# MAC-VO/MAC-VO

Measured on NVIDIA H100. Metric: stereo frames/sec @640x480, higher is better.
Workload: dtype f32

## Files before the change

include/macvo_b200.h:

```cpp
#ifndef MACVO_B200_H
#define MACVO_B200_H

#include <stddef.h>
#include <stdint.h>

#ifdef __cplusplus
extern "C" {
#endif

#define MACVO_OK 0
#define MACVO_E_ARG (-1)
#define MACVO_E_WORKSPACE (-2)
#define MACVO_E_UNSUPPORTED (-3)
#define MACVO_E_DRIVER (-4)

const char* macvo_b200_version(void);

#define MACVO_CORR_SIMT 0
#define MACVO_CORR_TC_3XF16 1
#define MACVO_CORR_TC_1XF16 2
#define MACVO_CORR_TC_TF32 3
#define MACVO_CORR_KMAJOR_INPUT 16
size_t macvo_corr_workspace_bytes(int batch, int dim, int n, int mode);
int macvo_corr_build(const float* fmap1, const float* fmap2, float* corr, int batch, int dim, int n, int mode,
// ... 50 lines not shown
                           float min_depth_cov, float match_cov_default, double* out_cov, float* out_point,
                           int* status, void* stream);

typedef struct {
    int max_steps;
    int patience;
    int max_reject;
    int cluster;
    double decreasing;
    double huber_delta;
    double radius;
    double diag_min;
    double diag_max;
} macvo_pgo_params_t;
int macvo_pgo_solve(const double* pos_Tw, const double* kp2_uv, const double* kp2_disp, const double* uv_cov,
                    const double* disp_cov, int k, const double* intr, double* pose_io,
                    const macvo_pgo_params_t* params, double* stats, void* stream);

#define MACVO_PGO_DISP 0
#define MACVO_PGO_REPROJ 1
#define MACVO_PGO_ICP 2
int macvo_pgo_solve_graph(int graph_type, const double* pos_Tw, const double* kp2_uv, const double* kp2_disp,
                          const double* uv_cov, const double* disp_cov, const double* pc_obs, const double* obs_cov,
                          const double* pts_cov, int k, const double* intr, double* pose_io,
                          const macvo_pgo_params_t* params, double* stats, void* stream);

int macvo_pgo_solve_counted(const double* pos_Tw, const double* kp2_uv, const double* kp2_disp, const double* uv_cov,
                            const double* disp_cov, int k_capacity, const int* k_dev, int min_k, const double* intr,
                            double* pose_io, const macvo_pgo_params_t* params, double* stats, void* stream,
                            int graph_type, const double* pc_obs, const double* obs_cov, const double* pts_cov);

size_t macvo_pgo_exchange_bytes(int world);
int macvo_p2p_alloc(size_t bytes, void** dev_ptr, unsigned char* ipc_handle64);
int macvo_p2p_open(const unsigned char* ipc_handle64, void** peer_ptr);
int macvo_p2p_close(void* peer_ptr);
int macvo_p2p_free(void* dev_ptr);
int macvo_pgo_solve_sharded(const double* pos_Tw, const double* kp2_uv, const double* kp2_disp, const double* uv_cov,
                            const double* disp_cov, int k_shard, const int* k_total_dev, int k_offset, int min_k,
                            const double* intr, double* pose_io, const macvo_pgo_params_t* params, double* stats,
                            void* const* exchange_bufs, int world, int rank, void* stream);

#define MACVO_PGO_ACC 55
#define MACVO_PGO_MAX_RANKS 8
int macvo_pgo_accumulate(const double* pos_Tw, const double* kp2_uv, const double* kp2_disp, const double* uv_cov,
                         const double* disp_cov, int k, const double* intr, const double* pose, double huber_delta,
                         double* acc, void* stream);

int macvo_layer_norm(const float* x, const float* weight, const float* bias, float* y, long long rows,
                     int channels, float eps, void* stream);
int macvo_add_layer_norm(const float* x, const float* resid, const float* weight, const float* bias, float* sum_out,
                         float* y, long long rows, int channels, float eps, void* stream);
int macvo_mlp_tc(const float* xn, const float* resid, const float* w1, const float* b1, const float* w2, const float* b2,
                 float* out, int rows, int channels, int hidden, void* stream);
int macvo_patch_embed_conv1(const float* maps, const float* weight, const float* bias, float* out,
                            long long n_maps, int h, int w, int allow_tf32, void* stream);
int macvo_add_rows_relu(float* x, const float* term, long long rows, int period, int channels, void* stream);
int macvo_small_attention(const float* q, const float* k, const float* v, float* out, int batch, int nq, int nk,
                          int heads, int head_dim, int q_broadcast, int allow_tf32, void* stream);

int macvo_small_attention_ex(const float* q, const float* k, const float* v, float* out, int batch, int nq, int nk,
                             int heads, int head_dim, int q_broadcast, int allow_tf32, int ldq, int ldk, int ldv,
                             const float* q_add, const float* k_add, int add_period, void* stream);

int macvo_latent_pool(const float* tokens, const float* ut, const float* wv, const float* bv, float* out,
                      long long n_maps, int nk, void* stream);

int macvo_gru_input(const float* mf, const float* agg, const float* gamma, float* buf0, float* buf1, float* buf2,
                    float* buf3, long long pixels, void* stream);
int macvo_gru_gates(const float* zr, const float* bias, const float* hx, float* z_out, float* rhx, long long pixels,
                    void* stream);
int macvo_gru_blend(const float* q, const float* bias, const float* z, float* hx, float* h_dense, long long pixels,
                    void* stream);
size_t macvo_rows_count(int batch, int height, int width, int vertical);
int macvo_conv_tc(const void* in_rows, int in_channels, int in_dense, const void* weights, const float* bias, int n_pad,
                  int n_valid, int ksize, int relu, int batch, int height, int width, void* out16, int out16_pitch,
                  int out16_offset, int out16_dense, float* out32, int out32_pitch, int out32_offset, int out32_planes,
                  void* stream);
int macvo_flow_im2col(const float* coords1, const float* coords0, void* rows, float* mf32, void* mf16_rows, int batch,
                      int height, int width, void* stream);

size_t macvo_gru_tc_operand_rows(int batch, int height, int width, int vertical);
int macvo_gru_tc_stage(int stage, int vertical, int batch, int height, int width, const void* h_rows, const void* x_rows,
                       const void* weights, const float* bias, float* h_master, float* z, void* out_rows, void* stream);
int macvo_gru_tc_pack(const float* src, int src_pitch, int channels, void* dst, int dst_channels, int dst_offset, int batch,
                      int height, int width, int vertical, void* stream);
int macvo_gru_tc_pack_motion(const float* mf, const float* agg, const float* gamma, void* x_rows_h, void* x_rows_v, int batch,
                             int height, int width, void* stream);
int macvo_softmax_rows_f16(const float* scores, void* out, long long rows, int cols, void* stream);
int macvo_convex_upsample(const float* flow, const float* mask_nhwc, float* out, float scale, int batch, int height, int width,
                          void* stream);

int macvo_cov_sanity_filter(const double* obs1_cov, const double* obs2_cov, int k, uint8_t* good, void* stream);
#define MACVO_COV_MATCH 0
#define MACVO_COV_IDENTITY 1
#define MACVO_COV_DIAGONALIZE 1
#define MACVO_COV_NORMALIZE 2
#define MACVO_COV_MAX_OPS 2
typedef struct {
    const float* depth_cov0;
    const float* depth_cov1;
    int simple_depth;
    float min_depth, max_depth;
    int front_of_cam;
    int icp;
    int cov_model;
    int cov_ops[MACVO_COV_MAX_OPS];
// ... 35 lines not shown
```

mac-vo_b200/build.py:

```python
from __future__ import annotations

import hashlib
import os
import shutil
import subprocess
import sys

PKG_DIR = os.path.dirname(os.path.abspath(__file__))
CSRC = os.path.join(PKG_DIR, "csrc")
LIB_DIR = os.path.join(PKG_DIR, "lib")
LIB_PATH = os.path.join(LIB_DIR, "libmacvo_b200.so")
SOURCES = ["corr_build.cu", "corr_build_simt.cu", "corr_build_tc.cu", "corr_lookup.cu", "dense_select.cu",
           "cov2to3.cu", "pgo.cu", "nn_kernels.cu", "decoder_fused.cu", "observe.cu", "decoder_token.cu", "motion_interp.cu",
           "gru_conv_tc.cu", "conv_tc.cu", "posenet.cu", "mlp_tc.cu"]
NVCC_FLAGS = ["-gencode", "arch=compute_90a,code=sm_90a", "-O3", "-lineinfo", "-std=c++17",
              "-Xcompiler", "-fPIC", "--use_fast_math=false"]


def _nvcc() -> str:
    for cand in (os.environ.get("NVCC"), shutil.which("nvcc"), "/usr/local/cuda/bin/nvcc"):
        if cand and os.path.exists(cand):
            return cand
    raise RuntimeError("nvcc not found (CUDA 12.9 toolkit expected at /usr/local/cuda)")


def _fingerprint() -> str:
    h = hashlib.sha256()
    for name in sorted(os.listdir(CSRC)) + ["../../include/macvo_b200.h"]:
        with open(os.path.join(CSRC, name), "rb") as f:
            h.update(name.encode())
            h.update(f.read())
    h.update(" ".join(NVCC_FLAGS).encode())
    return h.hexdigest()


def build(force: bool = False, verbose: bool = True) -> str:
    os.makedirs(LIB_DIR, exist_ok=True)
    stamp = os.path.join(LIB_DIR, "libmacvo_b200.stamp")
    fp = _fingerprint()
    if not force and os.path.exists(LIB_PATH) and os.path.exists(stamp) and open(stamp).read() == fp:
        return LIB_PATH
    nvcc = _nvcc()
    flags = [f for f in NVCC_FLAGS if f != "--use_fast_math=false"]
    objs = []
    procs = []
    for src in SOURCES:
        obj = os.path.join(LIB_DIR, src.replace(".cu", ".o"))
        objs.append(obj)
        cmd = [nvcc, *flags, "-c", os.path.join(CSRC, src), "-o", obj]
        procs.append((src, subprocess.Popen(cmd, stdout=subprocess.PIPE, stderr=subprocess.STDOUT, text=True)))
    for src, p in procs:
        out, _ = p.communicate()
        if p.returncode != 0:
            raise RuntimeError(f"nvcc failed on {src}:\n{out}")
        if verbose and out.strip():
            print(out, file=sys.stderr)
    link = [nvcc, "-shared", "-gencode", "arch=compute_90a,code=sm_90a", "-o", LIB_PATH, *objs, "-lcuda" if False else "-lcudart_static",
            "-Xlinker", "--no-undefined", "-lpthread", "-ldl", "-lrt"]
    r = subprocess.run(link, stdout=subprocess.PIPE, stderr=subprocess.STDOUT, text=True)
    if r.returncode != 0:
        raise RuntimeError(f"link failed:\n{r.stdout}")
    with open(stamp, "w") as f:
        f.write(fp)
    if verbose:
        print(f"built {LIB_PATH}", file=sys.stderr)
    return LIB_PATH

# ... 4 lines not shown
```

mac-vo_b200/csrc/nn_kernels.cu:

```cuda
#include "common.cuh"
#include <math_constants.h>

namespace {

__device__ __forceinline__ float2 ffma2_rn(float2 a, float2 b, float2 c) { return make_float2(fmaf(a.x, b.x, c.x), fmaf(a.y, b.y, c.y)); }
__device__ __forceinline__ float2 fmul2_rn(float2 a, float2 b) { return make_float2(__fmul_rn(a.x, b.x), __fmul_rn(a.y, b.y)); }

template <int VPL>
__global__ void __launch_bounds__(256)
layer_norm_kernel(const float* __restrict__ x, const float* __restrict__ w, const float* __restrict__ b,
                  float* __restrict__ y, long long rows, float eps, const float* __restrict__ resid = nullptr,
                  float* __restrict__ sum_out = nullptr) {
    constexpr int C = 32 * VPL;
    const long long row = (long long)blockIdx.x * 8 + (threadIdx.x >> 5);
    const int lane = threadIdx.x & 31;
    if (row >= rows) return;
    const float* xr = x + row * C;
    float v[VPL];
    float s = 0.f;
#pragma unroll
    for (int i = 0; i < VPL / 4; ++i) {
        float4 t = *reinterpret_cast<const float4*>(xr + (lane + 32 * i) * 4);
        if (resid) {
            const float4 r = *reinterpret_cast<const float4*>(resid + row * C + (lane + 32 * i) * 4);
            t = make_float4(t.x + r.x, t.y + r.y, t.z + r.z, t.w + r.w);
            *reinterpret_cast<float4*>(sum_out + row * C + (lane + 32 * i) * 4) = t;
        }
        v[4 * i] = t.x; v[4 * i + 1] = t.y; v[4 * i + 2] = t.z; v[4 * i + 3] = t.w;
        s += (t.x + t.y) + (t.z + t.w);
    }
    const float mean = warp_sum(s) * (1.f / C);
    float q = 0.f;
#pragma unroll
    for (int i = 0; i < VPL; ++i) { const float d = v[i] - mean; q = fmaf(d, d, q); }
    const float rstd = rsqrtf(warp_sum(q) * (1.f / C) + eps);
    float* yr = y + row * C;
#pragma unroll
    for (int i = 0; i < VPL / 4; ++i) {
        const int c = (lane + 32 * i) * 4;
        const float4 ww = *reinterpret_cast<const float4*>(w + c), bb = *reinterpret_cast<const float4*>(b + c);
        float4 o;
        o.x = (v[4 * i] - mean) * rstd * ww.x + bb.x;
        o.y = (v[4 * i + 1] - mean) * rstd * ww.y + bb.y;
        o.z = (v[4 * i + 2] - mean) * rstd * ww.z + bb.z;
        o.w = (v[4 * i + 3] - mean) * rstd * ww.w + bb.w;
        *reinterpret_cast<float4*>(yr + c) = o;
    }
}

__global__ void __launch_bounds__(256)
layer_norm64_kernel(const float* __restrict__ x, const float* __restrict__ w, const float* __restrict__ b,
                    float* __restrict__ y, long long rows, float eps) {
    const long long row = (long long)blockIdx.x * 8 + (threadIdx.x >> 5);
    const int lane = threadIdx.x & 31;
    if (row >= rows) return;
    const float2 t = *reinterpret_cast<const float2*>(x + row * 64 + lane * 2);
    const float mean = warp_sum(t.x + t.y) * (1.f / 64);
    const float d0 = t.x - mean, d1 = t.y - mean;
    const float rstd = rsqrtf(warp_sum(fmaf(d0, d0, d1 * d1)) * (1.f / 64) + eps);
    const float2 ww = *reinterpret_cast<const float2*>(w + lane * 2), bb = *reinterpret_cast<const float2*>(b + lane * 2);
    *reinterpret_cast<float2*>(y + row * 64 + lane * 2) = make_float2(d0 * rstd * ww.x + bb.x, d1 * rstd * ww.y + bb.y);
}

__global__ void __launch_bounds__(256)
add_rows_relu_kernel(float* __restrict__ x, const float* __restrict__ term, long long rows, int period, int c4) {
    const long long e = (long long)blockIdx.x * blockDim.x + threadIdx.x;
    if (e >= rows * c4) return;
    const long long r = e / c4;
    const int c = (int)(e % c4);
    float4 v = reinterpret_cast<float4*>(x)[e];
    const float4 t = __ldg(reinterpret_cast<const float4*>(term) + (r % period) * c4 + c);
    v.x = fmaxf(v.x + t.x, 0.f); v.y = fmaxf(v.y + t.y, 0.f); v.z = fmaxf(v.z + t.z, 0.f); v.w = fmaxf(v.w + t.w, 0.f);
    reinterpret_cast<float4*>(x)[e] = v;
}

constexpr int PE_C = 16, PE_K = 6;
__constant__ float c_pe_w[PE_K * PE_K * PE_C + PE_C];
__device__ float g_pe_pack[PE_K * PE_K * PE_C + PE_C];

__global__ void pe_pack_weights_kernel(const float* __restrict__ wgt, const float* __restrict__ bias, float* __restrict__ packed) {
    const int e = threadIdx.x + blockIdx.x * blockDim.x;
    if (e < PE_C * 36) { const int c = e / 36, t = e % 36; packed[t * PE_C + c] = wgt[e]; }
    else if (e < PE_C * 36 + PE_C) packed[e] = bias[e - PE_C * 36];
}

__global__ void __launch_bounds__(320)
patch_conv1_kernel(const float* __restrict__ maps, float* __restrict__ out, int h, int w, int ho, int wo) {
    extern __shared__ float sm[];
    float* s_map = sm;
    const int hp = 2 * ho + 4, wp = 2 * wo + 4;
    const float* src = maps + (long long)blockIdx.x * h * w;
    for (int e = threadIdx.x; e < hp * wp; e += blockDim.x) {
        const int y = e / wp - 2, x = e % wp - 2;
        s_map[e] = (y >= 0 && y < h && x >= 0 && x < w) ? __ldg(src + y * w + x) : 0.f;
    }
    __syncthreads();
    float* dst = out + (long long)blockIdx.x * ho * wo * PE_C;
    const int wo2 = wo >> 1;
    for (int p = threadIdx.x; p < ho * wo2; p += blockDim.x) {
        const int oy = p / wo2, ox = (p % wo2) * 2;
// ... 689 lines not shown
```

mac-vo_b200/flowformer_cov.py:

```python
from __future__ import annotations

import math
import os
import zlib
from typing import Callable

import torch
import torch.nn.functional as F

Tensor = torch.Tensor

LATENT_TOKENS = 8
LATENT_DIM = 128
QUERY_DIM = 64
COST_INPUT_DIM = 64
VERT_C_DIM = 64
ENCODER_DEPTH = 3


def _svt_spec(prefix: str) -> list[tuple[str, tuple[int, ...], str]]:
    out: list[tuple[str, tuple[int, ...], str]] = []
    dims, heads, srs, patch, cin = (128, 256), (4, 8), (8, 4), (4, 2), (3, 128)
    for s, (C, sr, ps, ci) in enumerate(zip(dims, srs, patch, cin)):
        p = f"{prefix}.svt."
# ... 312 lines not shown
        x = x.reshape(B, nh, nw, ws, ws, C).transpose(2, 3).reshape(B, nh * ws, nw * ws, C)
        return x[:, :H, :W, :].reshape(B, H * W, C)

    def _svt_local_attn(self, x: Tensor, size, p: str, heads: int, ws: int = 7) -> Tensor:
        B, N, C = x.shape
        H, W = size
        xw, meta = self._to_windows(x.view(B, H, W, C), ws)
        wq, bq = self.W[p + "qkv.weight"], self.W[p + "qkv.bias"]
        q, k, v = (F.linear(xw, wq[i * C:(i + 1) * C], bq[i * C:(i + 1) * C]) for i in range(3))
        o = self._attn(q, k, v, heads)
        return self._lin(self._from_windows(o, meta, ws, H, W), p + "proj")

    def _svt_global_attn(self, x: Tensor, size, p: str, heads: int, sr: int) -> Tensor:
        B, N, C = x.shape
        q = self._lin(x, p + "q")
        t = self._conv(x.permute(0, 2, 1).reshape(B, C, *size), p + "sr", stride=sr)
        t = self._ln(t.reshape(B, C, -1).permute(0, 2, 1), p + "norm")
        wkv, bkv = self.W[p + "kv.weight"], self.W[p + "kv.bias"]
        o = self._attn(q, F.linear(t, wkv[:C], bkv[:C]), F.linear(t, wkv[C:], bkv[C:]), heads)
        return self._lin(o, p + "proj")

    def patch_embed(self, cost_maps: Tensor) -> Tensor:
        p = "memory_encoder.cost_perceiver_encoder.patch_embed."
        M, _, H2, W2 = cost_maps.shape
        if self._native(cost_maps) and (H2 + 7) // 8 * 8 * ((W2 + 7) // 8 * 8) <= 96 * 160:
            if torch.backends.cudnn.allow_tf32:
                x = self._ops.patch_embed_conv1(cost_maps, self.W[p + "proj.0.weight"], self.W[p + "proj.0.bias"], s2d=True)
                w2 = self._memo(("pe_w2_s2d", x.device), lambda: self._ops.space_to_depth_filter(self.W[p + "proj.2.weight"])
                                .contiguous(memory_format=torch.channels_last))
                x = torch.cudnn_convolution_relu(x, w2, self.W[p + "proj.2.bias"], (1, 1), (1, 1), (1, 1), 1)
            else:
                x = self._ops.patch_embed_conv1(cost_maps, self.W[p + "proj.0.weight"], self.W[p + "proj.0.bias"])
                x = self._conv_relu(x, p + "proj.2", stride=2, padding=2)
        else:
            x = F.pad(cost_maps, (0, (8 - W2 % 8) % 8, 0, (8 - H2 % 8) % 8))
            x = self._conv_relu(x, p + "proj.0", stride=2, padding=2)
            x = self._conv_relu(x, p + "proj.2", stride=2, padding=2)
        native = self._native(x)
        x = F.conv2d(x if x.is_contiguous(memory_format=torch.channels_last) else x.contiguous(memory_format=torch.channels_last),
                     self.W[p + "proj.4.weight"], None if native else self.W[p + "proj.4.bias"], stride=2, padding=2)
        h, w = x.shape[2:]

        w0, b0 = self.W[p + "ffn_with_coord.0.weight"], self.W[p + "ffn_with_coord.0.bias"]

        def coord_term():
            xy = coords_grid(1, h, w, x.device, x.dtype) * 8 + 4
            enc = sine_embed(xy.view(1, 2, -1).permute(0, 2, 1), COST_INPUT_DIM)
            term = F.linear(enc, w0[:, COST_INPUT_DIM:, 0, 0], b0)
            if native:
                term = term + F.linear(self.W[p + "proj.4.bias"], w0[:, :COST_INPUT_DIM, 0, 0])
            return term.contiguous()
        term = self._memo(("pe", h, w, x.dtype, x.device, native), coord_term)
        t = x.permute(0, 2, 3, 1).reshape(M, h * w, COST_INPUT_DIM)
        t = F.linear(t, w0[:, :COST_INPUT_DIM, 0, 0])
        t = self._ops.add_rows_relu_(t, term[0]) if native else F.relu(t + term)
        t = F.linear(t, self.W[p + "ffn_with_coord.2.weight"][:, :, 0, 0], self.W[p + "ffn_with_coord.2.bias"])
        return self._ln(t, p + "norm")

    def _latent_layer(self, x: Tensor, p: str) -> Tensor:
        y = self._ln(x, p + "norm1")
        a = self._attn(self._lin(y, p + "q"), self._lin(y, p + "k"), self._lin(y, p + "v"), 8)
        x, xn = self._add_ln(x, self._lin(a, p + "proj"), p + "norm2")
        return self._mlp_residual(x, xn, p, "ffn.0", "ffn.3")

    def _context_tokens(self, context: Tensor, p: str, reps: int) -> Tensor:
        b, _, H, W = context.shape
        c = self._lin(context.flatten(2).permute(0, 2, 1), p + "context_proj").view(b, H, W, -1)
        return c.repeat(reps, 1, 1, 1)

    def _vert_local_attn_native(self, x: Tensor, size, context: Tensor, p: str, ws: int, heads: int) -> Tensor:
        Bt, N, C = x.shape
        H, W = size
        b = context.shape[0]
        wq, wk = self.W[p + "q.weight"], self.W[p + "k.weight"]
        enc = self._memo(("win", ws, C + VERT_C_DIM, x.dtype, x.device), lambda: sine_embed(
            coords_grid(1, ws, ws, x.device, x.dtype).view(1, 2, -1).permute(0, 2, 1), C + VERT_C_DIM))
        cproj = self._lin(context.flatten(2).permute(0, 2, 1), p + "context_proj").view(b, H, W, -1)
        cw, meta = self._to_windows(cproj, ws)
        w_qk_c = torch.cat([wq[:, C:], wk[:, C:]], 0)
        w_qk = torch.cat([wq, wk], 0)
        b_qk = torch.cat([self.W[p + "q.bias"], self.W[p + "k.bias"]], 0)
        terms = F.linear(cw, w_qk_c) + F.linear(enc, w_qk, b_qk)
        q_add, k_add = terms[..., :C].contiguous(), terms[..., C:].contiguous()
        w_x = self._memo(("vloc_w", p), lambda: torch.cat([wq[:, :C], wk[:, :C], self.W[p + "v.weight"]], 0).contiguous())
        b_x = self._memo(("vloc_b", p), lambda: torch.cat([torch.zeros(2 * C, device=x.device, dtype=x.dtype), self.W[p + "v.bias"]], 0))
        xw, meta = self._to_windows(x.view(Bt, H, W, C), ws)
        qkv = F.linear(xw, w_x, b_x)
        o = self._ops.fused_qkv_attention(qkv, heads, q_add, k_add)
        return self._lin(self._from_windows(o, meta, ws, H, W), p + "proj")

    def _vert_local_attn(self, x: Tensor, size, context: Tensor, p: str, ws: int = 7, heads: int = 8) -> Tensor:
        if self._native(x) and (x.shape[-1] // heads) in (16, 32):
            return self._vert_local_attn_native(x, size, context, p, ws, heads)
        Bt, N, C = x.shape
        H, W = size
        ctx = self._context_tokens(context, p, Bt // context.shape[0])
        xg = x.view(Bt, H, W, C)
        xw, meta = self._to_windows(xg, ws)
        qkw, _ = self._to_windows(torch.cat([xg, ctx], dim=-1), ws)
        enc = self._memo(("win", ws, C + VERT_C_DIM, x.dtype, x.device), lambda: sine_embed(
            coords_grid(1, ws, ws, x.device, x.dtype).view(1, 2, -1).permute(0, 2, 1), C + VERT_C_DIM))
        qkw = qkw + enc
        o = self._attn(self._lin(qkw, p + "q"), self._lin(qkw, p + "k"), self._lin(xw, p + "v"), heads)
        return self._lin(self._from_windows(o, meta, ws, H, W), p + "proj")

    def _vert_global_attn_native(self, x: Tensor, size, context: Tensor, p: str, sr: int, heads: int) -> Tensor:
        Bt, N, C = x.shape
        H, W = size
        b = context.shape[0]
# ... 414 lines not shown
```

mac-vo_b200/ops.py:

```python
from __future__ import annotations

import ctypes as C
import os
import threading

import torch

from .build import LIB_PATH

Tensor = torch.Tensor

CORR_SIMT, CORR_TC_3XF16, CORR_TC_1XF16, CORR_TC_TF32 = 0, 1, 2, 3
CORR_MODE_NAMES = {0: "simt", 1: "tc3", 2: "tc1", 3: "tf32"}
CORR_KMAJOR_INPUT = 16
PGO_ACC = 55

_lib = None
_lock = threading.Lock()
LAUNCHES = [0]


class MacvoB200Error(RuntimeError):
    pass

# ... 14 lines not shown
class _PgoParams(C.Structure):
    _fields_ = [("max_steps", C.c_int), ("patience", C.c_int), ("max_reject", C.c_int), ("cluster", C.c_int),
                ("decreasing", C.c_double), ("huber_delta", C.c_double), ("radius", C.c_double),
                ("diag_min", C.c_double), ("diag_max", C.c_double)]


EXPORTS = {
    "macvo_b200_version": (C.c_char_p, []),
    "macvo_corr_workspace_bytes": (C.c_size_t, [C.c_int] * 4),
    "macvo_corr_build": (C.c_int, [C.c_void_p] * 3 + [C.c_int] * 4 + [C.c_void_p, C.c_size_t, C.c_void_p]),
    "macvo_corr_lookup": (C.c_int, [C.c_void_p] * 3 + [C.c_int] * 5 + [C.c_void_p]),
    "macvo_corr_lookup_rows": (C.c_int, [C.c_void_p] * 3 + [C.c_int] * 5 + [C.c_void_p]),
    "macvo_dense_postproc": (C.c_int, [C.c_void_p] * 2 + [C.c_int] * 2 + [C.c_double] * 2 + [C.c_void_p] * 5
                             + [C.POINTER(_ScoreT), C.c_void_p]),
    "macvo_select_workspace_bytes": (C.c_size_t, [C.c_int] * 2),
    "macvo_select_candidates": (C.c_int, [C.c_void_p] * 5 + [C.c_int] * 3 + [C.c_double] + [C.c_void_p] * 5
                                + [C.c_size_t, C.c_void_p]),
    "macvo_select_candidates_depth": (C.c_int, [C.c_void_p] * 10 + [C.c_int] * 3 + [C.c_double] * 3 + [C.c_void_p] * 5
                                      + [C.c_size_t, C.c_void_p]),
    "macvo_select_mapping_candidates": (C.c_int, [C.c_void_p] * 2 + [C.c_int] * 3 + [C.c_float] * 2
                                        + [C.c_void_p] * 3 + [C.c_size_t, C.c_void_p]),
    "macvo_gather_pixels": (C.c_int, [C.c_void_p] * 2 + [C.c_int] * 2 + [C.c_void_p] * 2),
    "macvo_retrieve_pixels": (C.c_int, [C.c_void_p, C.c_int, C.c_int, C.c_void_p] + [C.c_int] * 3 + [C.c_void_p] * 2),
    "macvo_match_covariance": (C.c_int, [C.c_void_p, C.c_int, C.c_int, C.c_void_p, C.c_int, C.c_int, C.c_void_p,
                                         C.c_longlong, C.c_longlong, C.c_void_p]
                               + [C.c_float] * 4 + [C.c_int] + [C.c_float] * 3 + [C.c_void_p] * 4),
    "macvo_pgo_solve": (C.c_int, [C.c_void_p] * 5 + [C.c_int] + [C.c_void_p] * 2 + [C.POINTER(_PgoParams)]
                        + [C.c_void_p] * 2),
    "macvo_pgo_solve_graph": (C.c_int, [C.c_int] + [C.c_void_p] * 8 + [C.c_int] + [C.c_void_p] * 2 + [C.POINTER(_PgoParams)]
                              + [C.c_void_p] * 2),
    "macvo_pgo_solve_counted": (C.c_int, [C.c_void_p] * 5 + [C.c_int, C.c_void_p, C.c_int] + [C.c_void_p] * 2
                                + [C.POINTER(_PgoParams)] + [C.c_void_p] * 2 + [C.c_int] + [C.c_void_p] * 3),
    "macvo_motion_interpolate_workspace_bytes": (C.c_size_t, [C.c_int]),
    "macvo_motion_interpolate": (C.c_int, [C.c_void_p, C.c_void_p, C.c_int, C.c_void_p, C.c_void_p, C.c_size_t, C.c_void_p]),
    "macvo_cov_sanity_filter": (C.c_int, [C.c_void_p] * 2 + [C.c_int] + [C.c_void_p] * 2),
    "macvo_cov_modify": (C.c_int, [C.c_void_p, C.c_int, C.c_void_p, C.c_int, C.c_void_p]),
    "macvo_observe_workspace_bytes": (C.c_size_t, [C.c_int]),
    "macvo_observe_packed_doubles": (C.c_size_t, [C.c_int, C.c_int]),
    "macvo_observe_pack": (C.c_int, [C.c_void_p, C.c_int, C.c_int] + [C.c_void_p] * 6 + [C.c_int] * 3 + [C.c_void_p] * 2
                           + [C.c_int] + [C.c_float] * 3 + [C.c_void_p] * 6 + [C.c_size_t, C.c_void_p]
                           + [C.POINTER(_ObserveExt)]),
    "macvo_pgo_exchange_bytes": (C.c_size_t, [C.c_int]),
    "macvo_p2p_alloc": (C.c_int, [C.c_size_t, C.POINTER(C.c_void_p), C.c_char_p]),
    "macvo_p2p_open": (C.c_int, [C.c_char_p, C.POINTER(C.c_void_p)]),
    "macvo_p2p_close": (C.c_int, [C.c_void_p]),
    "macvo_p2p_free": (C.c_int, [C.c_void_p]),
    "macvo_pgo_solve_sharded": (C.c_int, [C.c_void_p] * 5 + [C.c_int, C.c_void_p, C.c_int, C.c_int] + [C.c_void_p] * 2
                                + [C.POINTER(_PgoParams)] + [C.c_void_p] * 2 + [C.c_int, C.c_int, C.c_void_p]),
    "macvo_pgo_accumulate": (C.c_int, [C.c_void_p] * 5 + [C.c_int] + [C.c_void_p] * 2 + [C.c_double]
                             + [C.c_void_p] * 2),
    "macvo_layer_norm": (C.c_int, [C.c_void_p] * 4 + [C.c_longlong, C.c_int, C.c_float, C.c_void_p]),
    "macvo_add_layer_norm": (C.c_int, [C.c_void_p] * 6 + [C.c_longlong, C.c_int, C.c_float, C.c_void_p]),
    "macvo_mlp_tc": (C.c_int, [C.c_void_p] * 7 + [C.c_int] * 3 + [C.c_void_p]),
    "macvo_patch_embed_conv1": (C.c_int, [C.c_void_p] * 4 + [C.c_longlong, C.c_int, C.c_int, C.c_int, C.c_void_p]),
    "macvo_add_rows_relu": (C.c_int, [C.c_void_p] * 2 + [C.c_longlong, C.c_int, C.c_int, C.c_void_p]),
    "macvo_small_attention": (C.c_int, [C.c_void_p] * 4 + [C.c_int] * 7 + [C.c_void_p]),
    "macvo_small_attention_ex": (C.c_int, [C.c_void_p] * 4 + [C.c_int] * 10 + [C.c_void_p] * 2 + [C.c_int, C.c_void_p]),
    "macvo_latent_pool": (C.c_int, [C.c_void_p] * 5 + [C.c_longlong, C.c_int, C.c_void_p]),
    "macvo_decoder_token_blob_floats": (C.c_size_t, []),
    "macvo_decoder_token": (C.c_int, [C.c_void_p] * 6 + [C.c_int, C.c_int, C.c_float, C.c_void_p]),
    "macvo_decoder_token_rows": (C.c_int, [C.c_void_p] * 6 + [C.c_int] * 3 + [C.c_float, C.c_void_p]),
    "macvo_gru_input": (C.c_int, [C.c_void_p] * 7 + [C.c_longlong, C.c_void_p]),
    "macvo_gru_gates": (C.c_int, [C.c_void_p] * 5 + [C.c_longlong, C.c_void_p]),
    "macvo_gru_blend": (C.c_int, [C.c_void_p] * 5 + [C.c_longlong, C.c_void_p]),
    "macvo_softmax_rows_f16": (C.c_int, [C.c_void_p] * 2 + [C.c_longlong, C.c_int, C.c_void_p]),
    "macvo_convex_upsample": (C.c_int, [C.c_void_p] * 3 + [C.c_float] + [C.c_int] * 3 + [C.c_void_p]),
    "macvo_rows_count": (C.c_size_t, [C.c_int] * 4),
    "macvo_conv_tc": (C.c_int, [C.c_void_p, C.c_int, C.c_int, C.c_void_p, C.c_void_p] + [C.c_int] * 7
                      + [C.c_void_p] + [C.c_int] * 3 + [C.c_void_p] + [C.c_int] * 3 + [C.c_void_p]),
    "macvo_flow_im2col": (C.c_int, [C.c_void_p] * 5 + [C.c_int] * 3 + [C.c_void_p]),
    "macvo_gru_tc_operand_rows": (C.c_size_t, [C.c_int] * 4),
    "macvo_gru_tc_stage": (C.c_int, [C.c_int] * 5 + [C.c_void_p] * 8),
    "macvo_gru_tc_pack": (C.c_int, [C.c_void_p, C.c_int, C.c_int, C.c_void_p] + [C.c_int] * 6 + [C.c_void_p]),
    "macvo_gru_tc_pack_motion": (C.c_int, [C.c_void_p] * 5 + [C.c_int] * 3 + [C.c_void_p]),
    "macvo_posenet_input": (C.c_int, [C.c_void_p] * 2 + [C.c_int] * 2 + [C.c_double, C.c_void_p, C.c_void_p]),
    "macvo_posenet_conv": (C.c_int, [C.c_void_p, C.c_int, C.c_int, C.c_int] + [C.c_void_p] * 2 + [C.c_int] * 5
                           + [C.c_void_p, C.c_int, C.c_void_p, C.c_void_p]),
    "macvo_posenet_head_floats": (C.c_size_t, []),
    "macvo_posenet_head": (C.c_int, [C.c_void_p] * 6),
}


def load_library(path: str | None = None):
    global _lib
    with _lock:
        if _lib is not None:
            return _lib
        path = path or os.environ.get("MACVO_B200_LIB", LIB_PATH)
        if not os.path.exists(path):
            raise MacvoB200Error(f"{path} not found: build it first with `python -m macvo_b200.build` "
                                 "(or __graft_entry__.build()); there is no CPU fallback")
        lib = C.CDLL(path)
        for name, (res, args) in EXPORTS.items():
            fn = getattr(lib, name)
            fn.restype, fn.argtypes = res, args
        _lib = lib
        return lib


def version() -> str:
    return load_library().macvo_b200_version().decode()


def _check(rc: int, what: str) -> None:
    if rc == 0:
        return
# ... 600 lines not shown
def layer_norm(x: Tensor, weight: Tensor, bias: Tensor, eps: float = 1e-5) -> Tensor:
    x = _dev(x, torch.float32, "layer_norm x")
    c = x.shape[-1]
    if c not in LAYER_NORM_CHANNELS:
        raise MacvoB200Error(f"layer_norm: channels {c} not in {LAYER_NORM_CHANNELS}")
    y = torch.empty_like(x)
    rc = load_library().macvo_layer_norm(x.data_ptr(), _dev(weight, torch.float32, "ln weight").data_ptr(),
                                         _dev(bias, torch.float32, "ln bias").data_ptr(), y.data_ptr(),
                                         x.numel() // c, c, float(eps), _stream())
    _check(rc, "macvo_layer_norm")
    LAUNCHES[0] += 1
    return y


def add_layer_norm(x: Tensor, resid: Tensor, weight: Tensor, bias: Tensor, eps: float = 1e-5) -> tuple[Tensor, Tensor]:
    x, resid = _dev(x, torch.float32, "add_layer_norm x"), _dev(resid, torch.float32, "add_layer_norm resid")
    c = x.shape[-1]
    if c not in (128, 256, 512) or x.shape != resid.shape:
        raise MacvoB200Error(f"add_layer_norm: channels {c} / shapes {tuple(x.shape)} vs {tuple(resid.shape)} unsupported")
    s, y = torch.empty_like(x), torch.empty_like(x)
    rc = load_library().macvo_add_layer_norm(x.data_ptr(), resid.data_ptr(), _dev(weight, torch.float32, "ln weight").data_ptr(),
                                             _dev(bias, torch.float32, "ln bias").data_ptr(), s.data_ptr(), y.data_ptr(),
                                             x.numel() // c, c, float(eps), _stream())
    _check(rc, "macvo_add_layer_norm")
    LAUNCHES[0] += 1
    return s, y


MLP_TC_HIDDEN = (128, 512)


def round_tf32(w: Tensor) -> Tensor:
    i = w.detach().to(torch.float32).contiguous().view(torch.int32)
    return ((i + 0xFFF + ((i >> 13) & 1)) & -0x2000).view(torch.float32)


def mlp_tc(xn: Tensor, resid: Tensor, w1: Tensor, b1: Tensor, w2: Tensor, b2: Tensor) -> Tensor:
    xn, resid = _dev(xn, torch.float32, "mlp_tc xn"), _dev(resid, torch.float32, "mlp_tc resid")
    w1, w2 = _dev(w1, torch.float32, "mlp_tc w1"), _dev(w2, torch.float32, "mlp_tc w2")
    b1, b2 = _dev(b1, torch.float32, "mlp_tc b1"), _dev(b2, torch.float32, "mlp_tc b2")
    c, hd = xn.shape[-1], w1.shape[0]
    if (c != 128 or hd not in MLP_TC_HIDDEN or xn.shape != resid.shape or tuple(w1.shape) != (hd, c)
            or tuple(w2.shape) != (c, hd) or b1.numel() != hd or b2.numel() != c):
        raise MacvoB200Error(f"mlp_tc: unsupported shapes xn {tuple(xn.shape)}, resid {tuple(resid.shape)}, "
                             f"w1 {tuple(w1.shape)}, w2 {tuple(w2.shape)}")
    out = torch.empty_like(resid)
    rc = load_library().macvo_mlp_tc(xn.data_ptr(), resid.data_ptr(), w1.data_ptr(), b1.data_ptr(), w2.data_ptr(),
                                      b2.data_ptr(), out.data_ptr(), xn.numel() // c, c, hd, _stream())
    _check(rc, "macvo_mlp_tc")
    LAUNCHES[0] += 1
    return out


def patch_embed_conv1(maps: Tensor, weight: Tensor, bias: Tensor, allow_tf32: bool | None = None, s2d: bool = False) -> Tensor:
    maps = _dev(maps, torch.float32, "patch_embed maps")
    m, one, h, w = maps.shape
    if one != 1 or tuple(weight.shape) != (16, 1, 6, 6):
        raise MacvoB200Error("patch_embed_conv1: expects (M,1,H,W) maps and a (16,1,6,6) weight")
    ho, wo = (h + 7) // 8 * 4, (w + 7) // 8 * 4
    tf32 = bool(torch.backends.cudnn.allow_tf32 if allow_tf32 is None else allow_tf32)
    if s2d and not tf32:
        raise MacvoB200Error("patch_embed_conv1: the space-to-depth output exists for the TF32 tensor-core variant only")
    out = torch.empty((m, ho // 2, wo // 2, 64) if s2d else (m, ho, wo, 16), dtype=torch.float32, device=maps.device)
    rc = load_library().macvo_patch_embed_conv1(maps.data_ptr(), _dev(weight, torch.float32, "w").data_ptr(),
                                                _dev(bias, torch.float32, "b").data_ptr(), out.data_ptr(),
                                                m, h, w, int(tf32) | (2 if s2d else 0), _stream())
    _check(rc, "macvo_patch_embed_conv1")
    LAUNCHES[0] += 1
    return out.permute(0, 3, 1, 2)


def space_to_depth_filter(weight: Tensor) -> Tensor:
    o, c, kh, kw = weight.shape
    if (kh, kw) != (6, 6):
        raise MacvoB200Error("space_to_depth_filter: expects a 6x6 filter")
    return weight.reshape(o, c, 3, 2, 3, 2).permute(0, 3, 5, 1, 2, 4).reshape(o, 4 * c, 3, 3)


def small_attention(q: Tensor, k: Tensor, v: Tensor, heads: int, allow_tf32: bool | None = None) -> Tensor:
    if allow_tf32 is None:
        allow_tf32 = bool(torch.backends.cuda.matmul.allow_tf32)
    q, k, v = (_dev(t, torch.float32, "attention operand") for t in (q, k, v))
    b, nk, c = k.shape
    d = c // heads
    nq = q.shape[1]
    if q.shape[0] not in (1, b) or q.shape[2] != c or v.shape != k.shape or d * heads != c:
        raise MacvoB200Error(f"small_attention: bad shapes q{tuple(q.shape)} k{tuple(k.shape)} v{tuple(v.shape)}")
    out = torch.empty(b, nq, c, dtype=torch.float32, device=k.device)
    rc = load_library().macvo_small_attention(q.data_ptr(), k.data_ptr(), v.data_ptr(), out.data_ptr(), b, nq, nk,
                                              heads, d, int(q.shape[0] == 1 and b > 1), int(allow_tf32), _stream())
    _check(rc, "macvo_small_attention")
    LAUNCHES[0] += 1
    return out


GRU_HID, GRU_IN = 128, 512


def _gru_buf(t: Tensor, what: str) -> Tensor:
    if not (t.is_cuda and t.dtype == torch.float32 and t.dim() == 2 and t.shape[1] == GRU_IN and t.is_contiguous()):
        raise MacvoB200Error(f"{what}: expected a contiguous fp32 CUDA (pixels, {GRU_IN}) buffer")
    return t


def gru_input(mf: Tensor, agg: Tensor, gamma: Tensor, bufs: list[Tensor]) -> None:
    mf, agg = _dense(mf, GRU_HID, "gru_input mf"), _dense(agg, GRU_HID, "gru_input agg")
# ... 408 lines not shown
```

Baseline: 46.13.

## Fuse patch-token FFN, coordinate term, ReLU and LayerNorm into one TF32 WGMMA kernel

Adds a persistent Hopper kernel that chains linear(64->128), an added coordinate term with ReLU, linear(128->128) with bias, and LayerNorm. It uses TMA loads and TF32 wgmma, and keeps the hidden activations in shared memory. This replaces two cuBLAS GEMMs plus separate add-relu and layer-norm launches, removing intermediate global-memory round trips and launch overhead. The path is taken only when native ops and TF32 matmul are enabled. The layer-norm math is moved into a shared header so the existing kernel can reuse it.

```diff
diff --git a/include/macvo_b200.h b/include/macvo_b200.h
--- a/include/macvo_b200.h
+++ b/include/macvo_b200.h
@@ -126,6 +126,9 @@
                          float* y, long long rows, int channels, float eps, void* stream);
 int macvo_mlp_tc(const float* xn, const float* resid, const float* w1, const float* b1, const float* w2, const float* b2,
                  float* out, int rows, int channels, int hidden, void* stream);
+int macvo_patch_tokens_tc(const float* x, const float* w0, const float* term, const float* w2, const float* b2,
+                          const float* ln_w, const float* ln_b, float* out, long long rows, int in_channels, int channels,
+                          int period, float eps, void* stream);
 int macvo_patch_embed_conv1(const float* maps, const float* weight, const float* bias, float* out,
                             long long n_maps, int h, int w, int allow_tf32, void* stream);
 int macvo_add_rows_relu(float* x, const float* term, long long rows, int period, int channels, void* stream);
diff --git a/mac-vo_b200/build.py b/mac-vo_b200/build.py
--- a/mac-vo_b200/build.py
+++ b/mac-vo_b200/build.py
@@ -12,7 +12,8 @@
 LIB_PATH = os.path.join(LIB_DIR, "libmacvo_b200.so")
 SOURCES = ["corr_build.cu", "corr_build_simt.cu", "corr_build_tc.cu", "corr_lookup.cu", "dense_select.cu",
            "cov2to3.cu", "pgo.cu", "nn_kernels.cu", "decoder_fused.cu", "observe.cu", "decoder_token.cu", "motion_interp.cu",
-           "gru_conv_tc.cu", "conv_tc.cu", "posenet.cu", "mlp_tc.cu"]
+           "gru_conv_tc.cu", "conv_tc.cu", "posenet.cu", "mlp_tc.cu",
+           "patch_tokens_tc.cu"]
 NVCC_FLAGS = ["-gencode", "arch=compute_90a,code=sm_90a", "-O3", "-lineinfo", "-std=c++17",
               "-Xcompiler", "-fPIC", "--use_fast_math=false"]
 
diff --git a/mac-vo_b200/csrc/layer_norm_row.cuh b/mac-vo_b200/csrc/layer_norm_row.cuh
--- /dev/null
+++ b/mac-vo_b200/csrc/layer_norm_row.cuh
@@ -0,0 +1,25 @@
+#pragma once
+#include "common.cuh"
+
+template <int VPL>
+__device__ __forceinline__ void layer_norm_row(float (&v)[VPL], const float* __restrict__ w, const float* __restrict__ b,
+                                               float eps, int lane) {
+    constexpr int C = 32 * VPL;
+    float s = 0.f;
+#pragma unroll
+    for (int i = 0; i < VPL / 4; ++i) s += (v[4 * i] + v[4 * i + 1]) + (v[4 * i + 2] + v[4 * i + 3]);
+    const float mean = warp_sum(s) * (1.f / C);
+    float q = 0.f;
+#pragma unroll
+    for (int i = 0; i < VPL; ++i) { const float d = v[i] - mean; q = fmaf(d, d, q); }
+    const float rstd = rsqrtf(warp_sum(q) * (1.f / C) + eps);
+#pragma unroll
+    for (int i = 0; i < VPL / 4; ++i) {
+        const int c = (lane + 32 * i) * 4;
+        const float4 ww = *reinterpret_cast<const float4*>(w + c), bb = *reinterpret_cast<const float4*>(b + c);
+        v[4 * i] = (v[4 * i] - mean) * rstd * ww.x + bb.x;
+        v[4 * i + 1] = (v[4 * i + 1] - mean) * rstd * ww.y + bb.y;
+        v[4 * i + 2] = (v[4 * i + 2] - mean) * rstd * ww.z + bb.z;
+        v[4 * i + 3] = (v[4 * i + 3] - mean) * rstd * ww.w + bb.w;
+    }
+}
diff --git a/mac-vo_b200/csrc/nn_kernels.cu b/mac-vo_b200/csrc/nn_kernels.cu
--- a/mac-vo_b200/csrc/nn_kernels.cu
+++ b/mac-vo_b200/csrc/nn_kernels.cu
@@ -1,4 +1,5 @@
 #include "common.cuh"
+#include "layer_norm_row.cuh"
 #include <math_constants.h>
 
 namespace {
@@ -17,7 +18,6 @@
     if (row >= rows) return;
     const float* xr = x + row * C;
     float v[VPL];
-    float s = 0.f;
 #pragma unroll
     for (int i = 0; i < VPL / 4; ++i) {
         float4 t = *reinterpret_cast<const float4*>(xr + (lane + 32 * i) * 4);
@@ -27,25 +27,12 @@
             *reinterpret_cast<float4*>(sum_out + row * C + (lane + 32 * i) * 4) = t;
         }
         v[4 * i] = t.x; v[4 * i + 1] = t.y; v[4 * i + 2] = t.z; v[4 * i + 3] = t.w;
-        s += (t.x + t.y) + (t.z + t.w);
-    }
-    const float mean = warp_sum(s) * (1.f / C);
-    float q = 0.f;
-#pragma unroll
-    for (int i = 0; i < VPL; ++i) { const float d = v[i] - mean; q = fmaf(d, d, q); }
-    const float rstd = rsqrtf(warp_sum(q) * (1.f / C) + eps);
+    }
+    layer_norm_row<VPL>(v, w, b, eps, lane);
     float* yr = y + row * C;
 #pragma unroll
-    for (int i = 0; i < VPL / 4; ++i) {
-        const int c = (lane + 32 * i) * 4;
-        const float4 ww = *reinterpret_cast<const float4*>(w + c), bb = *reinterpret_cast<const float4*>(b + c);
-        float4 o;
-        o.x = (v[4 * i] - mean) * rstd * ww.x + bb.x;
-        o.y = (v[4 * i + 1] - mean) * rstd * ww.y + bb.y;
-        o.z = (v[4 * i + 2] - mean) * rstd * ww.z + bb.z;
-        o.w = (v[4 * i + 3] - mean) * rstd * ww.w + bb.w;
-        *reinterpret_cast<float4*>(yr + c) = o;
-    }
+    for (int i = 0; i < VPL / 4; ++i)
+        *reinterpret_cast<float4*>(yr + (lane + 32 * i) * 4) = make_float4(v[4 * i], v[4 * i + 1], v[4 * i + 2], v[4 * i + 3]);
 }
 
 __global__ void __launch_bounds__(256)
diff --git a/mac-vo_b200/csrc/patch_tokens_tc.cu b/mac-vo_b200/csrc/patch_tokens_tc.cu
--- /dev/null
+++ b/mac-vo_b200/csrc/patch_tokens_tc.cu
@@ -0,0 +1,199 @@
+#include "tc_common.cuh"
+#include "layer_norm_row.cuh"
+
+namespace {
+
+constexpr int PT_IN = 64, PT_C = 128, PT_ROWS = 128;
+constexpr int X_SUB = PT_ROWS * 128;
+constexpr int X_BYTES = 2 * X_SUB;
+constexpr int W0_SUB = PT_C * 128;
+constexpr int W0_BYTES = 2 * W0_SUB;
+constexpr int W2_SUB = PT_C * 128;
+constexpr int W2_BYTES = 4 * W2_SUB;
+constexpr int HID_SUB = 64 * 128;
+constexpr int HID_WG_BYTES = 4 * HID_SUB;
+constexpr int OFF_W2 = W0_BYTES, OFF_X = OFF_W2 + W2_BYTES, OFF_HID = OFF_X + 2 * X_BYTES;
+constexpr int OFF_BAR = OFF_HID + 2 * HID_WG_BYTES;
+constexpr int PT_SMEM = OFF_BAR + 64 + 1024;
+static_assert(PT_SMEM <= 227 * 1024, "shared memory budget");
+static_assert(PT_ROWS * PT_C * 4 == 2 * HID_WG_BYTES, "the pre-norm rows reuse the hidden tiles");
+
+constexpr uint32_t SW128_DESC_HI = (1024u >> 4) | (1u << 30);
+__device__ __forceinline__ uint32_t sw128_lo(uint32_t smem_addr) { return ((smem_addr & 0x3FFFFu) >> 4) | (1u << 16); }
+__device__ __forceinline__ uint64_t sw128_desc(uint32_t lo) { return ((uint64_t)SW128_DESC_HI << 32) | lo; }
+
+__device__ __forceinline__ uint32_t to_tf32(float x) {
+    uint32_t r;
+    asm("cvt.rn.tf32.f32 %0, %1;" : "=r"(r) : "f"(x));
+    return r;
+}
+
+__device__ __forceinline__ void wg_sync(int wg) {
+    if (wg == 0) asm volatile("bar.sync 2, 128;" ::: "memory");
+    else asm volatile("bar.sync 3, 128;" ::: "memory");
+}
+
+__global__ void __launch_bounds__(TC_THREADS, 1)
+patch_tokens_tc_kernel(const __grid_constant__ CUtensorMap map_x, const __grid_constant__ CUtensorMap map_w0,
+                       const __grid_constant__ CUtensorMap map_w2, const float* __restrict__ term, const float* __restrict__ b2,
+                       const float* __restrict__ ln_w, const float* __restrict__ ln_b, float* __restrict__ out, int rows,
+                       int period, float eps) {
+    extern __shared__ uint8_t smem_raw[];
+    uint8_t* smem = reinterpret_cast<uint8_t*>((reinterpret_cast<uintptr_t>(smem_raw) + 1023) & ~(uintptr_t)1023);
+    const uint32_t s_base = smem_u32(smem);
+    const uint32_t bar_w = s_base + OFF_BAR, bar_xf = bar_w + 8, bar_xe = bar_xf + 16;
+    const int warp = threadIdx.x >> 5, lane = threadIdx.x & 31;
+    const int tiles = ceil_div(rows, PT_ROWS);
+
+    if (threadIdx.x == 0) {
+        mbar_init(bar_w, 1);
+        for (int s = 0; s < 2; ++s) { mbar_init(bar_xf + 8 * s, 1); mbar_init(bar_xe + 8 * s, 2); }
+        fence_barrier_init();
+        prefetch_tmap(&map_x); prefetch_tmap(&map_w0); prefetch_tmap(&map_w2);
+    }
+    __syncthreads();
+
+    if (warp == TC_PRODUCER_WARP) {
+        if (elect_one()) {
+            mbar_expect_tx(bar_w, W0_BYTES + W2_BYTES);
+            for (int kc = 0; kc < 2; ++kc) tma_load_2d(s_base + kc * W0_SUB, &map_w0, bar_w, 32 * kc, 0);
+            for (int kc = 0; kc < 4; ++kc) tma_load_2d(s_base + OFF_W2 + kc * W2_SUB, &map_w2, bar_w, 32 * kc, 0);
+            int it = 0;
+            for (int t = blockIdx.x; t < tiles; t += gridDim.x, ++it) {
+                const int s = it & 1;
+                mbar_wait(bar_xe + 8 * s, ((it >> 1) & 1) ^ 1);
+                mbar_expect_tx(bar_xf + 8 * s, X_BYTES);
+                for (int kc = 0; kc < 2; ++kc) tma_load_2d(s_base + OFF_X + s * X_BYTES + kc * X_SUB, &map_x, bar_xf + 8 * s, 32 * kc, t * PT_ROWS);
+            }
+        }
+        return;
+    }
+
+    const int wg = warp >> 2, t128 = threadIdx.x & 127;
+    const bool leader = t128 == 0;
+    const uint32_t hid = s_base + OFF_HID + wg * HID_WG_BYTES;
+    const int fr = (warp & 3) * 16 + (lane >> 2), fc = 2 * (lane & 3);
+    float acc[64];
+
+    mbar_wait(bar_w, 0);
+    int it = 0;
+    for (int t = blockIdx.x; t < tiles; t += gridDim.x, ++it) {
+        const int s = it & 1;
+        const uint32_t xs = s_base + OFF_X + s * X_BYTES;
+        mbar_wait(bar_xf + 8 * s, (it >> 1) & 1);
+#pragma unroll
+        for (int kc = 0; kc < 2; ++kc) {
+#pragma unroll
+            for (int u = 0; u < 4; ++u) {
+                const uint32_t a = xs + kc * X_SUB + wg * 64 * 128 + (u * 128 + t128) * 16;
+                const float4 v = lds128(a);
+                asm volatile("st.shared.v4.b32 [%0], {%1, %2, %3, %4};" ::"r"(a), "r"(to_tf32(v.x)), "r"(to_tf32(v.y)),
+                             "r"(to_tf32(v.z)), "r"(to_tf32(v.w)) : "memory");
+            }
+        }
+        asm volatile("fence.proxy.async.shared::cta;" ::: "memory");
+        wg_sync(wg);
+
+        {
+            uint32_t xd = sw128_lo(xs + wg * 64 * 128), wd = sw128_lo(s_base);
+            asm volatile("" : "+r"(xd), "+r"(wd));
+            wgmma_fence();
+#pragma unroll
+            for (int kc = 0; kc < 2; ++kc) {
+#pragma unroll
+                for (int k = 0; k < 4; ++k)
+                    Wgmma<128>::tf32(acc, sw128_desc(xd + (kc * X_SUB >> 4) + 2 * k), sw128_desc(wd + (kc * W0_SUB >> 4) + 2 * k),
+                                     (kc | k) != 0);
+            }
+            wgmma_commit();
+            wgmma_wait<0>();
+            fence_acc(acc);
+        }
+        if (leader) mbar_arrive(bar_xe + 8 * s);
+
+        {
+            const int row0 = t * PT_ROWS + wg * 64 + fr;
+            const float* tr0 = term + (long long)(row0 % period) * PT_C;
+            const float* tr1 = term + (long long)((row0 + 8) % period) * PT_C;
+#pragma unroll
+            for (int i = 0; i < 64; i += 2) {
+                const int r = fr + 8 * ((i >> 1) & 1), c = 8 * (i >> 2) + fc;
+                const float2 tt = __ldg(reinterpret_cast<const float2*>(((i >> 1) & 1 ? tr1 : tr0) + c));
+                const uint32_t v0 = to_tf32(fmaxf(acc[i] + tt.x, 0.f)), v1 = to_tf32(fmaxf(acc[i + 1] + tt.y, 0.f));
+                const int cc = c & 31;
+                const uint32_t addr = hid + (c >> 5) * HID_SUB + r * 128 + ((((cc >> 2) ^ (r & 7))) << 4) + (cc & 3) * 4;
+                asm volatile("st.shared.v2.b32 [%0], {%1, %2};" ::"r"(addr), "r"(v0), "r"(v1) : "memory");
+            }
+        }
+        asm volatile("fence.proxy.async.shared::cta;" ::: "memory");
+        wg_sync(wg);
+
+        {
+            uint32_t hd = sw128_lo(hid), wd = sw128_lo(s_base + OFF_W2);
+            asm volatile("" : "+r"(hd), "+r"(wd));
+            wgmma_fence();
+#pragma unroll
+            for (int kc = 0; kc < 4; ++kc) {
+#pragma unroll
+                for (int k = 0; k < 4; ++k)
+                    Wgmma<128>::tf32(acc, sw128_desc(hd + (kc * HID_SUB >> 4) + 2 * k), sw128_desc(wd + (kc * W2_SUB >> 4) + 2 * k),
+                                     (kc | k) != 0);
+            }
+            wgmma_commit();
+            wgmma_wait<0>();
+            fence_acc(acc);
+        }
+
+        wg_sync(wg);
+#pragma unroll
+        for (int i = 0; i < 64; i += 2) {
+            const float2 bb = __ldg(reinterpret_cast<const float2*>(b2 + 8 * (i >> 2) + fc));
+            acc[i] = acc[i] + bb.x;
+            acc[i + 1] = acc[i + 1] + bb.y;
+        }
+        stage_acc_rows<128>(hid, PT_C * 4, acc, 0);
+        wg_sync(wg);
+
+        const int wrow0 = t * PT_ROWS + wg * 64 + (warp & 3) * 16;
+#pragma unroll 2
+        for (int j = 0; j < 16; ++j) {
+            const int r = (warp & 3) * 16 + j;
+            const float4 x4 = lds128(hid + r * (PT_C * 4) + ((lane ^ (r & 7)) << 4));
+            float v[4] = {x4.x, x4.y, x4.z, x4.w};
+            layer_norm_row<4>(v, ln_w, ln_b, eps, lane);
+            if (wrow0 + j < rows)
+                __stcs(reinterpret_cast<float4*>(out + (long long)(wrow0 + j) * PT_C) + lane, make_float4(v[0], v[1], v[2], v[3]));
+        }
+    }
+}
+
+}
+
+int macvo_patch_tokens_tc(const float* x, const float* w0, const float* term, const float* w2, const float* b2,
+                          const float* ln_w, const float* ln_b, float* out, long long rows, int in_channels, int channels,
+                          int period, float eps, void* stream) {
+    if (!x || !w0 || !term || !w2 || !b2 || !ln_w || !ln_b || !out || rows < 0 || period <= 0) return MACVO_E_ARG;
+    if (in_channels != PT_IN || channels != PT_C || rows > (long long)INT32_MAX - PT_ROWS) return MACVO_E_UNSUPPORTED;
+    for (const void* p : {(const void*)x, (const void*)w0, (const void*)term, (const void*)w2, (const void*)b2,
+                          (const void*)ln_w, (const void*)ln_b, (const void*)out})
+        if (reinterpret_cast<uintptr_t>(p) & 15) return MACVO_E_ARG;
+    if (rows == 0) return MACVO_OK;
+    CUtensorMap m_x, m_w0, m_w2;
+    bool ok = make_map_2d(&m_x, CU_TENSOR_MAP_DATA_TYPE_FLOAT32, 4, x, PT_IN, (uint64_t)rows, PT_IN * 4, 32, PT_ROWS);
+    ok = ok && make_map_2d(&m_w0, CU_TENSOR_MAP_DATA_TYPE_FLOAT32, 4, w0, PT_IN, PT_C, PT_IN * 4, 32, PT_C);
+    ok = ok && make_map_2d(&m_w2, CU_TENSOR_MAP_DATA_TYPE_FLOAT32, 4, w2, PT_C, PT_C, PT_C * 4, 32, PT_C);
+    if (!ok) return MACVO_E_DRIVER;
+    static int sms = 0;
+    if (!sms) {
+        int dev = 0, n = 0;
+        MACVO_CUDA_TRY(cudaGetDevice(&dev));
+        MACVO_CUDA_TRY(cudaDeviceGetAttribute(&n, cudaDevAttrMultiProcessorCount, dev));
+        MACVO_CUDA_TRY(cudaFuncSetAttribute(patch_tokens_tc_kernel, cudaFuncAttributeMaxDynamicSharedMemorySize, PT_SMEM));
+        sms = n;
+    }
+    const int tiles = ceil_div((int)rows, PT_ROWS);
+    patch_tokens_tc_kernel<<<tiles < sms ? tiles : sms, TC_THREADS, PT_SMEM, as_stream(stream)>>>(
+        m_x, m_w0, m_w2, term, b2, ln_w, ln_b, out, (int)rows, period, eps);
+    MACVO_LAUNCH_CHECK();
+    return MACVO_OK;
+}
diff --git a/mac-vo_b200/flowformer_cov.py b/mac-vo_b200/flowformer_cov.py
--- a/mac-vo_b200/flowformer_cov.py
+++ b/mac-vo_b200/flowformer_cov.py
@@ -388,9 +388,15 @@
             return term.contiguous()
         term = self._memo(("pe", h, w, x.dtype, x.device, native), coord_term)
         t = x.permute(0, 2, 3, 1).reshape(M, h * w, COST_INPUT_DIM)
+        w2 = self.W[p + "ffn_with_coord.2.weight"][:, :, 0, 0]
+        if native and torch.backends.cuda.matmul.allow_tf32:
+            w0t, w2t = self._memo(("pe_tc", x.device), lambda: (self._ops.round_tf32(w0[:, :COST_INPUT_DIM, 0, 0]),
+                                                                self._ops.round_tf32(w2)))
+            return self._ops.patch_tokens_tc(t, w0t, term[0], w2t, self.W[p + "ffn_with_coord.2.bias"],
+                                             self.W[p + "norm.weight"], self.W[p + "norm.bias"])
         t = F.linear(t, w0[:, :COST_INPUT_DIM, 0, 0])
         t = self._ops.add_rows_relu_(t, term[0]) if native else F.relu(t + term)
-        t = F.linear(t, self.W[p + "ffn_with_coord.2.weight"][:, :, 0, 0], self.W[p + "ffn_with_coord.2.bias"])
+        t = F.linear(t, w2, self.W[p + "ffn_with_coord.2.bias"])
         return self._ln(t, p + "norm")
 
     def _latent_layer(self, x: Tensor, p: str) -> Tensor:
diff --git a/mac-vo_b200/ops.py b/mac-vo_b200/ops.py
--- a/mac-vo_b200/ops.py
+++ b/mac-vo_b200/ops.py
@@ -90,6 +90,7 @@
     "macvo_layer_norm": (C.c_int, [C.c_void_p] * 4 + [C.c_longlong, C.c_int, C.c_float, C.c_void_p]),
     "macvo_add_layer_norm": (C.c_int, [C.c_void_p] * 6 + [C.c_longlong, C.c_int, C.c_float, C.c_void_p]),
     "macvo_mlp_tc": (C.c_int, [C.c_void_p] * 7 + [C.c_int] * 3 + [C.c_void_p]),
+    "macvo_patch_tokens_tc": (C.c_int, [C.c_void_p] * 8 + [C.c_longlong, C.c_int, C.c_int, C.c_int, C.c_float, C.c_void_p]),
     "macvo_patch_embed_conv1": (C.c_int, [C.c_void_p] * 4 + [C.c_longlong, C.c_int, C.c_int, C.c_int, C.c_void_p]),
     "macvo_add_rows_relu": (C.c_int, [C.c_void_p] * 2 + [C.c_longlong, C.c_int, C.c_int, C.c_void_p]),
     "macvo_small_attention": (C.c_int, [C.c_void_p] * 4 + [C.c_int] * 7 + [C.c_void_p]),
@@ -796,6 +797,26 @@
     return out
 
 
+def patch_tokens_tc(x: Tensor, w0: Tensor, term: Tensor, w2: Tensor, b2: Tensor, ln_w: Tensor, ln_b: Tensor,
+                    eps: float = 1e-5) -> Tensor:
+    x, term = _dev(x, torch.float32, "patch_tokens_tc x"), _dev(term, torch.float32, "patch_tokens_tc term")
+    w0, w2 = _dev(w0, torch.float32, "patch_tokens_tc w0"), _dev(w2, torch.float32, "patch_tokens_tc w2")
+    b2 = _dev(b2, torch.float32, "patch_tokens_tc b2")
+    ln_w, ln_b = _dev(ln_w, torch.float32, "patch_tokens_tc ln_w"), _dev(ln_b, torch.float32, "patch_tokens_tc ln_b")
+    cin, c = x.shape[-1], w0.shape[0]
+    if (cin != 64 or c != 128 or tuple(w0.shape) != (c, cin) or tuple(w2.shape) != (c, c) or term.dim() != 2
+            or term.shape[1] != c or term.shape[0] == 0 or any(t.numel() != c for t in (b2, ln_w, ln_b))):
+        raise MacvoB200Error(f"patch_tokens_tc: unsupported shapes x {tuple(x.shape)}, w0 {tuple(w0.shape)}, "
+                             f"term {tuple(term.shape)}, w2 {tuple(w2.shape)}")
+    out = torch.empty(*x.shape[:-1], c, dtype=torch.float32, device=x.device)
+    rc = load_library().macvo_patch_tokens_tc(x.data_ptr(), w0.data_ptr(), term.data_ptr(), w2.data_ptr(), b2.data_ptr(),
+                                              ln_w.data_ptr(), ln_b.data_ptr(), out.data_ptr(), x.numel() // cin, cin, c,
+                                              term.shape[0], float(eps), _stream())
+    _check(rc, "macvo_patch_tokens_tc")
+    LAUNCHES[0] += 1
+    return out
+
+
 def patch_embed_conv1(maps: Tensor, weight: Tensor, bias: Tensor, allow_tf32: bool | None = None, s2d: bool = False) -> Tensor:
     maps = _dev(maps, torch.float32, "patch_embed maps")
     m, one, h, w = maps.shape
```

After: 47.62 (median of 6 runs). 1.03x the previous value.
